# patrickltobing/cyclevae-vc

Measured on AMD Instinct MI355X. Metric: mcep_frames_per_sec_hu1024_ld32_cyc2, higher is better.
Workload: dtype f32 (every matrix product on exact fp32 operands: each operand carried as three fp16 limbs x = l0 + l1/2^11 + l2/2^22, six v_mfma_f32_32x32x16_f16 per product, f32 accumulate; dropped terms < 2^-33 of a product; gates, carried state, projection and outputs f32)

## Files before the change

cyclevae-vc_amd/csrc/cvae_kernels.h:

```cpp
#pragma once
#include <cvae_intrin.h>
#include <stdint.h>

struct CvaeSeg {
    const float* ptr;
    int width;
    int row_stride;
};

__device__ __forceinline__ void cvae_philox(uint32_t c0, uint32_t c1, uint32_t c2, uint32_t c3, uint32_t k0,
                                            uint32_t k1, uint32_t out[4]) {
    for (int i = 0; i < 10; ++i) {
        const uint64_t p0 = (uint64_t)0xD2511F53u * c0, p1 = (uint64_t)0xCD9E8D57u * c2;
        const uint32_t n0 = (uint32_t)(p1 >> 32) ^ c1 ^ k0, n1 = (uint32_t)p1;
        const uint32_t n2 = (uint32_t)(p0 >> 32) ^ c3 ^ k1, n3 = (uint32_t)p0;
        c0 = n0; c1 = n1; c2 = n2; c3 = n3;
        k0 += 0x9E3779B9u; k1 += 0xBB67AE85u;
    }
    out[0] = c0; out[1] = c1; out[2] = c2; out[3] = c3;
}

__device__ __forceinline__ void cvae_randn_pair(uint32_t w0, uint32_t w1, float& zc, float& zs) {
    const float u1 = ((float)(w0 >> 8) + 0.5f) * (1.0f / 16777216.0f);
    const float u2 = ((float)(w1 >> 8) + 0.5f) * (1.0f / 16777216.0f);
// ... 165 lines not shown
#define CVAE_MAX_CELLS 32
struct ProParams {
    ProCell cell[CVAE_MAX_CELLS];
    int ncell, L;
    uint64_t frame0;
    const float* sin_w;
    const float* sin_b;
    const float* wo;
    const float* bo;
    int B, T, C, Cp, pad, Co, H, Bp, nslack, nzero;
    long mtot;
    float* xnp;
    float* hbuf;
    float* hx;
    float* xt;
    int nxt_slack;
    float* hs;
    float* xs;
    long xs_plane;
    float* dy;
    unsigned* zero_words;
    int* zero_status;
    int zero_status_n;
    unsigned* ll_counter;
    int nA, nH, nD;
    int nG;
    float* gx0;
    const float* wyT;
    int* range_word;
    int* range_epoch;
    int range_val;
    float range_at;
    const int* image_unfit;
};
#ifndef CVAE_STATUS_RANGE_WORD
#define CVAE_STATUS_RANGE_WORD 3
#endif
#define CVAE_WS_RANGE_WORD 20
#define CVAE_WS_RANGE_EPOCH 21
#define CVAE_LIMB_MAX 65504.0f
__device__ __forceinline__ bool cvae_out_of_range(float v, float bound) { return !(fabsf(v) < bound); }
__device__ __forceinline__ void cvae_flag_unfit(int* unfit, float w) {
    if (cvae_out_of_range(w, CVAE_LIMB_MAX)) *unfit = 1;
}
static_assert(sizeof(ProParams) <= 4096, "ProParams is a kernel argument: 4 KiB at most");

__device__ __forceinline__ float cvae_input_value(const ProParams& p, const ProCell& c, int b, int t, int q, const float* emean = nullptr) {
    const long fr = (long)b * p.T + t;
    if (q < c.seg0.width) return c.seg0.ptr[fr * c.seg0.row_stride + q];
    if (!c.lat) return c.seg1.ptr[fr * c.seg1.row_stride + (q - c.seg0.width)];
    const int l = q - c.seg0.width;
    float e;
    if (c.n_draws > 1 && emean) {
        e = emean[l];
    } else if (c.n_draws > 1) {
        e = 0.0f;
        const long es = c.eps_stride ? c.eps_stride : (long)p.B * p.T * p.L;
        for (int k = 0; k < c.n_draws; ++k)
            e += c.eps ? c.eps[(long)k * es + fr * p.L + l]
                       : cvae_randn(c.seed, c.draw + (uint64_t)k, (uint64_t)(fr + c.draw_frame0) + p.frame0, (uint32_t)l);
        e *= 1.0f / (float)c.n_draws;
    } else {
        e = c.eps ? c.eps[fr * p.L + l] : cvae_randn(c.seed, c.draw, (uint64_t)(fr + c.draw_frame0) + p.frame0, (uint32_t)l);
    }
    return c.lat[fr * 2 * p.L + l] + expf(c.lat[fr * 2 * p.L + p.L + l] * 0.5f) * e;
}

__device__ __forceinline__ void cvae_mean_draws(const ProParams& p, const ProCell& c, int b, int t, float* part, float* emean) {
    const int tid = threadIdx.x, L = p.L, nq = L >> 2, nsl = 256 / nq, qd = tid % nq, sl = tid / nq;
    const long fr = (long)b * p.T + t;
    const long es = c.eps_stride ? c.eps_stride : (long)p.B * p.T * p.L;
    if (sl < nsl) {
        float e[4] = {0.f, 0.f, 0.f, 0.f};
        for (int k = sl; k < c.n_draws; k += nsl) {
            float z[4];
            if (c.eps) {
                const float* ep = c.eps + (long)k * es + fr * p.L + 4 * qd;
                z[0] = ep[0]; z[1] = ep[1]; z[2] = ep[2]; z[3] = ep[3];
            } else {
                cvae_randn4(c.seed, c.draw + (uint64_t)k, (uint64_t)(fr + c.draw_frame0) + p.frame0, (uint32_t)qd, z);
            }
#pragma unroll
            for (int j = 0; j < 4; ++j) e[j] += z[j];
        }
#pragma unroll
        for (int j = 0; j < 4; ++j) part[sl * L + 4 * qd + j] = e[j];
    }
    __syncthreads();
    if (tid < L) {
        float m = 0.0f;
        for (int q = 0; q < nsl; ++q) m += part[q * L + tid];
        emean[tid] = m * (1.0f / (float)c.n_draws);
    }
    __syncthreads();
}

__global__ void k_prologue(ProParams p) {
    const int tid = threadIdx.x, blk = blockIdx.x;
    const int Tp = p.T + 2 * p.pad;
    if (blk < p.nA && p.xt) {
        float* raw = (float*)CVAE_SMEM;
        unsigned char* img = (unsigned char*)(raw + 32 * (p.C + 1));
        const int tile = blk / Tp, tp = blk % Tp, t = tp - p.pad, np = p.Cp >> 3;
        float* tmean = (float*)(img + np * 1280);
        const bool quads = p.L > 0 && (p.L & 3) == 0;
        if (quads) {
            const int nq = p.L >> 2;
            for (int item = tid; item < 32 * nq; item += 256) {
                const int r = item / nq, qd = item - r * nq, bb = tile * 32 + r;
                if (bb >= p.ncell * p.B) continue;
                const ProCell& c = p.cell[bb / p.B];
                if (!c.lat || c.n_draws <= 1 || !CVAE_FRAME_VALID(p, c, t)) continue;
                const long fr = (long)(bb % p.B) * p.T + t, es = c.eps_stride ? c.eps_stride : (long)p.B * p.T * p.L;
                float e[4] = {0.f, 0.f, 0.f, 0.f};
                for (int k = 0; k < c.n_draws; ++k) {
                    float z[4];
                    if (c.eps) {
                        const float* ep = c.eps + (long)k * es + fr * p.L + 4 * qd;
                        z[0] = ep[0]; z[1] = ep[1]; z[2] = ep[2]; z[3] = ep[3];
                    } else {
                        cvae_randn4(c.seed, c.draw + (uint64_t)k, (uint64_t)(fr + c.draw_frame0) + p.frame0, (uint32_t)qd, z);
                    }
#pragma unroll
                    for (int j = 0; j < 4; ++j) e[j] += z[j];
                }
#pragma unroll
                for (int j = 0; j < 4; ++j) tmean[r * p.L + 4 * qd + j] = e[j] * (1.0f / (float)c.n_draws);
            }
            __syncthreads();
        }
        for (int idx = tid; idx < 32 * p.C; idx += 256) {
            const int r = idx / p.C, q = idx - r * p.C, bb = tile * 32 + r;
            float v = 0.0f;
            if (bb < p.ncell * p.B) {
                const ProCell& c = p.cell[bb / p.B];
                if (CVAE_FRAME_VALID(p, c, t)) v = cvae_input_value(p, c, bb % p.B, t, q, quads ? tmean + r * p.L : nullptr);
            }
            raw[r * (p.C + 1) + q] = v;
        }
        __syncthreads();
        const ProCell* const cells = p.cell;
        bool bad = false;
        for (int q = tid & 63; q < p.Cp; q += 64) {
            float v[8];
            bool ok[8];
#pragma unroll
            for (int i = 0; i < 8; ++i) {
                const int r = (tid >> 6) + 4 * i, bb = tile * 32 + r;
                ok[i] = false;
                if (bb < p.ncell * p.B) {
                    const ProCell& c = cells[bb / p.B];
                    ok[i] = CVAE_FRAME_VALID(p, c, t) && q < p.C;
                }
                v[i] = !ok[i] ? 0.0f : (p.sin_w ? p.sin_b[q] : raw[r * (p.C + 1) + q]);
            }
            if (p.sin_w && q < p.C)
                for (int k = 0; k < p.C; ++k) {
                    const float w = p.sin_w[(long)q * p.C + k];
#pragma unroll
                    for (int i = 0; i < 8; ++i) v[i] += w * raw[((tid >> 6) + 4 * i) * (p.C + 1) + k];
                }
            unsigned char* pc = img + (q >> 3) * 1280;
#pragma unroll
            for (int i = 0; i < 8; ++i) {
                const int r = (tid >> 6) + 4 * i;
                unsigned short l0, l1;
                unsigned char l2;
                cvae_split3_f16b8(ok[i] ? v[i] : 0.0f, l0, l1, l2);
                bad = bad || (ok[i] && cvae_out_of_range(v[i], p.range_at));
                ((unsigned short*)pc)[r * 8 + (q & 7)] = l0;
                ((unsigned short*)(pc + 512))[r * 8 + (q & 7)] = l1;
                pc[1024 + r * 8 + (q & 7)] = l2;
            }
        }
        const bool fits = cvae_block_all(!bad);
        if (!fits && p.range_word && tid == 0) *p.range_word = p.range_val;
        f32x4* dst = (f32x4*)((unsigned char*)p.xt + ((long)tile * Tp + tp) * np * 1280);
        for (int e = tid; e < np * 80; e += 256) dst[e] = ((const f32x4*)img)[e];
        return;
    }
    if (p.nG > 0 && blk >= p.nA + p.nH + p.nD && blk < p.nA + p.nH + p.nD + p.nG) {
        const long q4 = ((long)(blk - p.nA - p.nH - p.nD) * blockDim.x + tid) * 4, H3 = 3L * p.H;
        if (q4 < (long)p.ncell * p.B * H3) {
            const int bb = (int)(q4 / H3), col = (int)(q4 - (long)bb * H3);
            const float* yi = p.cell[bb / p.B].y_in + (long)(bb % p.B) * p.Co;
            float a0 = 0.f, a1 = 0.f, a2 = 0.f, a3 = 0.f;
            int c = 0;
            for (; c + 8 <= p.Co; c += 8) {
                float d[8], w[8][4];
#pragma unroll
                for (int q = 0; q < 8; ++q) {
                    d[q] = yi[c + q] - p.bo[c + q];
                    const float* wp = p.wyT + (long)(c + q) * H3 + col;
                    w[q][0] = wp[0]; w[q][1] = wp[1]; w[q][2] = wp[2]; w[q][3] = wp[3];
                }
#pragma unroll
                for (int q = 0; q < 8; ++q) { a0 += w[q][0] * d[q]; a1 += w[q][1] * d[q]; a2 += w[q][2] * d[q]; a3 += w[q][3] * d[q]; }
            }
            for (; c < p.Co; ++c) {
                const float d = yi[c] - p.bo[c];
                const float* w = p.wyT + (long)c * H3 + col;
                a0 += w[0] * d; a1 += w[1] * d; a2 += w[2] * d; a3 += w[3] * d;
            }
            float* o = p.gx0 + (long)bb * H3 + col;
            o[0] = a0; o[1] = a1; o[2] = a2; o[3] = a3;
        }
        return;
    }
    const float* emean = nullptr;
    if (blk < p.nA && blockDim.x == 256) {
        const int tp = blk % Tp, bb = blk / Tp, t = tp - p.pad;
        if (bb < p.ncell * p.B) {
            const ProCell& c = p.cell[bb / p.B];
            if (c.lat && c.n_draws > 1 && p.L <= 256 && (p.L & 3) == 0 && CVAE_FRAME_VALID(p, c, t)) {
                float* part = (float*)CVAE_SMEM + p.C;
// ... 1040 lines not shown
```

cyclevae-vc_amd/csrc/cvae_lib.hip:

```cpp
#include <cvae_intrin.h>

#include <stdarg.h>
#include <stdio.h>
#include <stdlib.h>
#include <string.h>

#include <atomic>
#include <map>
#include <mutex>
#include <new>
#include <utility>
#include <vector>

#include "cvae_kernels.h"
#include "cvae_train_kernels.h"
#include "cvae_deep.h"
#include "cyclevae_hip.h"

namespace {

thread_local char g_err[512] = "";

enum OptId {
    OPT_V6_LIMBS_H64, OPT_NO_LL, OPT_MAX_RT, OPT_LL_BACKOFF, OPT_EXP, OPT_GEMM_FORCE, OPT_GEMM_LOG, OPT_TRAIN_OLD_GEMM,
    OPT_GEMM_TRACE, OPT_TRAIN_PER_STEP, OPT_TRAIN_PROF, OPT_TRAIN_BACKOFF, OPT_TRAIN_FP32_MFMA, OPT_TRAIN_BWD_PER_STEP, OPT_TRAIN_KERNEL, OPT_X3_TILE, OPT_BWD_OVERFLOW_AT, OPT_GEMM_MAX_SPLIT, OPT_BWD_KS, OPT_COOP_LAUNCH, OPT_V6_LIMBS_H2048, OPT_V6_W2S_H64, OPT_STEP_COL_TILES, OPT_TRAIN_PROFILE, OPT_TRAIN_XMAP, OPT_MASKS_ON_SIDE, OPT_V6_BACKOFF, OPT_TRAIN_BWD_BACKOFF, OPT_LL_ROW_PAD, OPT_GEMM_MIN_DEPTH, OPT_TRAIN_BWD_GEOM, OPT_BWD_W3_L1_H64, OPT_TRAIN_FWD_GEOM, OPT_TRAIN_FWD_BACKOFF, OPT_EXACT_RANGE_AT, OPT_DTW_BATCH_COST, OPT_COUNT
};
struct OptEntry { const char* name; long dflt; };
const OptEntry g_opt[OPT_COUNT] = {
    {"v6_limbs_h64", 3},
    {"no_ll", 0},
    {"max_rt", 0},
    {"ll_backoff", -1},
    {"exp", 0},
    {"gemm_force", 0},
    {"gemm_log", 0},
    {"train_old_gemm", 0},
    {"gemm_trace", 0},
    {"train_per_step", 0},
    {"train_prof", 0},
    {"train_backoff", 32},
    {"train_fp32_mfma", 0},
    {"train_bwd_per_step", 0},
    {"train_kernel", 0},
    {"x3_tile", 0},
    {"bwd_overflow_at", 60000},
    {"gemm_max_split", 16},
    {"bwd_ks", 8},
    {"coop_launch", 0},
    {"v6_limbs_h2048", 3},
    {"v6_w2s_h64", 0},
    {"step_col_tiles", 0},
    {"train_profile", 0},
    {"train_xmap", 0},
    {"masks_on_side", 1},
    {"v6_backoff", -1},
    {"train_bwd_backoff", -1},
    {"ll_row_pad", 0},
    {"gemm_min_depth", 128},
    {"train_bwd_geom", -1},
    {"bwd_w3_l1_h64", 0},
    {"train_fwd_geom", -1},
    {"train_fwd_backoff", -1},
    {"exact_range_at", 65504},
    {"dtw_batch_cost", 1},
};

struct ProfEvents {
    std::vector<hipEvent_t> start, stop;
    std::vector<int> rows, cin;
    size_t used = 0;
};
enum { TPROF_FWD = 0, TPROF_BWD = 1, TPROF_GEMM = 2, TPROF_WGRAD = 3, TPROF_CLASSES = 4 };
struct TrainProfEvents {
    std::vector<hipEvent_t> start, stop;
    std::vector<int> cls;
    std::vector<double> flop;
    size_t used = 0;
};
struct SideDone { const void* scratch; hipEvent_t ev; };

}

struct cvae_ctx {
    int32_t* status_sink = nullptr;
    long draw_row0 = 0, draw_rows = 0, draw_frames = 0, draw_parts = 1;
    long opt[OPT_COUNT];
    ProfEvents prof;
    TrainProfEvents tprof;
    hipStream_t side = nullptr;
    SideDone side_done[8] = {};
    hipEvent_t side_ready = nullptr, side_join = nullptr, side_last = nullptr;
    int side_cap = 0;
    hipEvent_t mask_fork = nullptr, mask_join = nullptr;
    unsigned side_evict = 0;
    int32_t* gemm_ran = nullptr;
    std::map<const void*, std::pair<int, unsigned long>> train_var;
    unsigned long train_var_tick = 0;
// ... 416 lines not shown
        const cvae_pass_input* in = cells[c].in;
        const int w_in = in->seg0.width + (in->lat ? in->lat_dim : in->seg1.width);
        if (w_in != m.C) return fail(-1, "cell %d: pass input width %d != in_dim %d", c, w_in, m.C);
        if (in->frames < 0 || in->frames > T) return fail(-1, "cell %d: frames %d outside [0, T=%d]", c, in->frames, T);
        if (in->ctx_before < 0 || in->ctx_after < 0 || in->draw_frame0 < 0 || in->eps_draw_stride < 0)
            return fail(-1, "cell %d: negative window context / draw origin", c);
        if ((in->ctx_before || in->ctx_after || in->draw_frame0) && B != 1)
            return fail(-1, "cell %d: windows of a longer utterance (ctx_before / ctx_after / draw_frame0) are single-row cells, B=%d", c, B);
    }
    return 0;
}

struct ProTargets {
    int shape;
    float* xnp;
    float* dy;
    float* slot0;
    unsigned* zero_words;
    int nzero;
    int* zero_status;
    int zero_status_n;
    int* ws_status;
    bool limbs, new_call;
    float* hx;
    float* xt;
    int nxt_slack;
    float* hs;
    float* xs;
    long xs_plane;
    float* gx0;
    unsigned* ll_counter;
};
struct RangeSlot { int* word; int val; float at; };

void run_prologue(const Dims& m, const cvae_net_desc* d, const float* P, const Prep& pl, const PassRows& r, const ProTargets& o,
                  hipStream_t st, RangeSlot* range = nullptr) {
    const Cell* cells = r.cells;
    const int ncell = r.ncell, B = r.B, T = r.T, Bp = r.Bp, shape = o.shape;
    const int Brows = ncell * B, Tp = T + 2 * m.pad;
    ProParams pp;
    memset(&pp, 0, sizeof(pp));
    for (int c = 0; c < ncell; ++c) {
        const cvae_pass_input* in = cells[c].in;
        pp.cell[c].seg0 = CvaeSeg{in->seg0.ptr, in->seg0.width, in->seg0.row_stride};
        pp.cell[c].seg1 = CvaeSeg{in->seg1.ptr, in->seg1.width, in->seg1.row_stride};
        pp.cell[c].lat = in->lat;
        pp.cell[c].eps = in->eps;
        pp.cell[c].seed = in->seed;
        pp.cell[c].draw = in->draw_id;
        pp.cell[c].y_in = cells[c].y_in;
        pp.cell[c].h_in = cells[c].h_in;
        pp.cell[c].frames = in->frames;
        pp.cell[c].n_draws = in->n_draws;
        pp.cell[c].ctx_before = in->ctx_before; pp.cell[c].ctx_after = in->ctx_after;
        pp.cell[c].draw_frame0 = (long)in->draw_frame0; pp.cell[c].eps_stride = (long)in->eps_draw_stride;
        if (in->lat) pp.L = in->lat_dim;
    }
    pp.ncell = ncell;
    pp.frame0 = (uint64_t)cx().draw_row0 * (uint64_t)T;
    pp.sin_w = d->has_scale_in ? P + pl.sin_w : nullptr;
    pp.sin_b = d->has_scale_in ? P + pl.sin_b : nullptr;
    pp.wo = P + pl.wo; pp.bo = P + pl.bo;
    pp.B = B; pp.T = T; pp.C = m.C; pp.Cp = m.Cp; pp.pad = m.pad; pp.Co = m.Co; pp.H = m.H; pp.Bp = Bp;
    pp.nslack = 64 * m.KFW + 64;
    pp.mtot = r.mtot;
    pp.xnp = o.xnp; pp.hbuf = o.slot0; pp.dy = o.dy;
    pp.hx = o.hx; pp.xt = o.xt; pp.nxt_slack = o.nxt_slack;
    pp.hs = o.hs; pp.xs = o.xs; pp.xs_plane = o.xs_plane;
    pp.zero_words = o.zero_words; pp.nzero = o.nzero;
    pp.zero_status = o.zero_status; pp.zero_status_n = o.zero_status_n;
    pp.ll_counter = o.ll_counter;
    pp.nA = (shape == PRO_TILES ? Bp / 32 : Brows) * Tp;
    pp.nH = (int)nblk((long)Bp * m.H, 1024);
    pp.nD = (int)nblk((long)Brows * m.Co, 64);
    pp.nG = o.gx0 ? (int)nblk((long)Brows * m.H3 / 4, shape == PRO_ROWS ? 64 : 256) : 0;
    pp.gx0 = o.gx0; pp.wyT = P + pl.wyT;
    range_params(pp, o.ws_status, o.limbs, o.new_call, P, pl);
    if (range) *range = RangeSlot{pp.range_word, pp.range_val, pp.range_at};
    const dim3 gp(pp.nA + pp.nH + pp.nD + pp.nG + 1);
    if (shape == PRO_TILES)
        hipLaunchKernelGGL((k_prologue), gp, dim3(256),
                           (size_t)32 * (m.C + 1) * sizeof(float) + (size_t)(m.Cp / 8) * 1280 + (size_t)32 * pp.L * sizeof(float), st, pp);
    else if (shape == PRO_DRAWS)
        hipLaunchKernelGGL((k_prologue), gp, dim3(256), (size_t)(m.C + 1024 + 256) * sizeof(float), st, pp);
    else
        hipLaunchKernelGGL((k_prologue), gp, dim3(64), m.C * sizeof(float), st, pp);
}

void run_front_end_gemm(const Dims& m, const float* P, const Prep& pl, const float* xnp, float* gx, int rows, int Tp, hipStream_t st) {
    const int M = rows * Tp, N = m.H3;
    hipLaunchKernelGGL((k_gemm_nt<4, 4, 2, 2, false>), dim3(nblk(N, 128), nblk(M, 128)), dim3(256), 0, st, xnp, (long)m.Cp, 0L,
                       P + pl.afold, (long)m.Kfe, P + pl.cfold, gx, (long)m.H3, M, N, m.Kfe);
}

void run_projection(const Dims& m, const cvae_net_desc* d, const float* P, const Prep& pl, const PassRows& r, int proj, const float* hbuf,
                    float* y, int clamp_lat_dim, hipStream_t st) {
    const Cell* cells = r.cells;
    const int ncell = r.ncell, B = r.B, T = r.T, Bp = r.Bp;
    const long mtot = r.mtot;
    if (proj == PROJ_FUSED) {
        OutParams op;
        op.hbuf = hbuf; op.mtot = mtot; op.wo2 = P + pl.wo2; op.bo2 = P + pl.bo2; op.H = m.H; op.Bp = Bp; op.T = T;
        op.B = B; op.ncell = ncell; op.Co = m.Co; op.clamp_from = d->has_scale_out ? -1 : clamp_dim(clamp_lat_dim);
        op.clamp_min = clamp_floor(clamp_lat_dim);
        for (int c = 0; c < CVAE_MAX_CELLS; ++c) op.out[c] = c < ncell ? cells[c].trj_out : nullptr;
        const int ntn = m.Cop / 16;
        const unsigned nb = (unsigned)((long)T * Bp / 16);
        const size_t lds = (size_t)4 * 16 * (m.Cop + 4) * sizeof(float);
        void (*const kout)(OutParams) = ntn == 1 ? k_outproj<1> : ntn == 4 ? k_outproj<4> : k_outproj<8>;
        hipLaunchKernelGGL(kout, dim3(nb), dim3(256), lds, st, op);
        return;
    }
    const int M = T * Bp, N = m.Co;
    hipLaunchKernelGGL((k_gemm_nt<2, 4, 4, 1, true>), dim3(nblk(N, 64), nblk(M, 128)), dim3(256), 0, st, hbuf + (long)Bp * 16, 0L, mtot,
                       P + pl.wo, (long)m.H, P + pl.bo, y, (long)m.Cop, M, N, m.H);
    for (int c = 0; c < ncell; ++c) {
        EpiParams ep;
        ep.y = y; ep.ldy = m.Cop;
        ep.sout_w = d->has_scale_out ? P + pl.sout_w : nullptr;
        ep.sout_b = d->has_scale_out ? P + pl.sout_b : nullptr;
        ep.clamp_from = d->has_scale_out ? -1 : clamp_dim(clamp_lat_dim);
        ep.clamp_min = clamp_floor(clamp_lat_dim);
        ep.B = B; ep.Bp = Bp; ep.T = T; ep.Co = m.Co; ep.b0 = c * B;
        ep.trj_out = cells[c].trj_out; ep.y_last = cells[c].y_last;
        ep.t_last = last_slot(cells[c].in, T) - 1;
        hipLaunchKernelGGL((k_epilogue), dim3(B * T), dim3(64), m.Co * sizeof(float), st, ep);
    }
}

void run_last_states(const Dims& m, const PassRows& r, const float* hbuf, hipStream_t st) {
    for (int c = 0; c < r.ncell; ++c)
        if (r.cells[c].h_last)
            hipLaunchKernelGGL((k_hlast), dim3(nblk((long)r.B * m.H, 256)), dim3(256), 0, st, hbuf, r.mtot, r.cells[c].h_last, r.B, r.Bp,
                               m.H, last_slot(r.cells[c].in, r.T), c * r.B);
}

int run_pass(const Dims& m, const cvae_net_desc* d, const float* P, const Cell* cells, int ncell, int B, int T,
             int clamp_lat_dim, float* ws, int* status, int flags, hipStream_t st, bool clear_status = false) {
    const Prep pl = prep_layout(m, d->has_scale_in != 0, d->has_scale_out != 0);
    const int Brows = ncell * B;
    const Work wl = work_layout(m, Brows, T);
    int* const ws_status = status;
    if (cx().status_sink) status = cx().status_sink;
    const PassRows rows = {cells, ncell, B, T, wl.Bp, wl.mtot};
    if (int rc = check_cells(m, rows)) return rc;
    unsigned* bar = (unsigned*)(ws + wl.status) + 8;
    float* xnp = ws + wl.xnp;
    float* gx = ws + wl.gx;
    float* hbuf = ws + wl.hbuf;
    float* dy = ws + wl.dy;
    unsigned* hflags = (unsigned*)(ws + wl.flags);
    long long* const step_prof = (flags & CVAE_FLAG_STEP_TIMING) ? (long long*)(ws + wl.prof) : nullptr;
    const int cus = cu_count();
    PassFacts facts = {};
    for (int c = 0; c < ncell; ++c) {
        facts.h_in = facts.h_in || cells[c].h_in != nullptr;
        facts.y_last = facts.y_last || cells[c].y_last != nullptr;
        facts.h_last = facts.h_last || cells[c].h_last != nullptr;
        facts.many_draws = facts.many_draws || (cells[c].in->lat && cells[c].in->n_draws > 1);
    }
    const EvalPlan pn = plan_eval_pass(m, Brows, T, flags, cus, image_known_unfit(P), facts);

    {
        ProTargets o = {};
        o.shape = pn.prologue; o.xnp = xnp; o.dy = dy;
        o.slot0 = hbuf;
        o.zero_words = hflags; o.nzero = wl.Bp / 16 * m.nch;
        o.zero_status = clear_status ? status : nullptr;
        o.zero_status_n = cx().status_sink ? 4 : 8;
        o.ws_status = ws_status; o.limbs = pn.limbs; o.new_call = clear_status;
        const bool triples = pn.form == CVAE_EVAL_V6 || pn.form == CVAE_EVAL_V6H;
        o.hx = triples ? ws + wl.hs : nullptr;
        o.xt = pn.form == CVAE_EVAL_V6 ? ws + wl.xt : nullptr;
        o.nxt_slack = (int)wl.xt_slack;
        o.hs = pn.pairs ? ws + wl.hs : nullptr;
        o.xs = pn.pairs ? ws + wl.xs : nullptr;
        o.xs_plane = wl.xs_plane;
        o.gx0 = pn.gx0_ready ? ws + wl.gx0 : nullptr;
        o.ll_counter = pn.form == CVAE_EVAL_LL ? (unsigned*)(ws + wl.status) + 16 : nullptr;
        run_prologue(m, d, P, pl, rows, o, st);
    }

    const size_t lds2 = (4 * 16 * 84 + 16 * 16) * sizeof(float);
    const bool prof = (flags & CVAE_FLAG_PROFILE) && prof_begin(st, ncell * B, m.C);
    const auto refused = [](hipError_t e) {
        if (e == hipSuccess) return false;
        (void)hipGetLastError();
        return true;
    };
    int form = pn.form;
    if (form == CVAE_EVAL_LL || form == CVAE_EVAL_V6H || form <= CVAE_EVAL_V2) run_front_end_gemm(m, P, pl, xnp, gx, Brows, wl.Tp, st);
    switch (form) {
    case CVAE_EVAL_LL: {
        StepLLParams q;
        q.hbuf = hbuf; q.mtot = wl.mtot; q.xbuf = ws + wl.hs; q.wrec2 = P + pl.wrec2; q.gx = gx; q.gx_bstride = (long)wl.Tp * m.H3;
        q.bhn = P + pl.bhn; q.B = Brows; q.Bp = wl.Bp; q.H = m.H; q.T = T; q.status = status;
        q.prof = step_prof;
        q.wyT = P + pl.wyT; q.dy = dy; q.Co = m.Co;
        q.dbg = (int*)(ws + wl.status);
        q.backoff = pn.backoff;
        q.nonce_src = (const unsigned*)(ws + wl.status) + 16;
        const dim3 gl(m.H / 4);
        const size_t ldsl = (size_t)(2 * 64 * 49 + 4 * 48) * sizeof(float);
        const hipError_t e = cvae_launch_coop(Brows == 1 ? k_gru_steps_ll<1> : Brows == 2 ? k_gru_steps_ll<2> : k_gru_steps_ll<3>, gl,
                                              dim3(256), ldsl, st, q);
        if (refused(e)) return fail(-3, "small-batch recurrent kernel failed to launch: %s", hipGetErrorString(e));
        break;
    }
    case CVAE_EVAL_V6:
    case CVAE_EVAL_V6H: {
        const bool fused = form == CVAE_EVAL_V6;
        Step6Params q;
        q.hbuf = hbuf; q.mtot = wl.mtot; q.hx = ws + wl.hs; q.wrec3 = P + pl.wrec_t; q.afold3 = fused ? P + pl.afold_t : nullptr; q.w2s = P + pl.wrec_l2b;
        q.cfold = P + pl.cfold; q.bhn = P + pl.bhn; q.xt = fused ? ws + wl.xt : nullptr; q.Tp = wl.Tp; q.Cp = m.Cp;
        q.gx = fused ? nullptr : gx; q.gx_bstride = (long)wl.Tp * m.H3;
        q.B = Brows; q.Bp = wl.Bp; q.H = m.H; q.T = T; q.flags = hflags; q.status = status;
        q.prof = step_prof;
        q.wyT = P + pl.wyT; q.dy = dy; q.Co = m.Co;
        q.gx0 = pn.gx0_ready ? ws + wl.gx0 : nullptr;
        q.want_f32 = pn.want_f32 ? 1 : 0;
        q.rts = pn.rts;
        q.exp = (int)opt(OPT_EXP);
        q.backoff = pn.backoff;
        const size_t lds6 = (size_t)(4 * 32 * 40 + 32 * 8 + 384 + (fused ? 4 * m.KFW * v6_limbs(m) * 256 : 0)) * sizeof(float);
        const hipError_t e = cvae_launch_coop(pn.k6, dim3(m.H / 8 * pn.rts), dim3(256), lds6, st, q);
        if (refused(e)) return fail(-3, "exact-operand recurrent kernel failed to launch: %s", hipGetErrorString(e));
        break;
    }
    case CVAE_EVAL_V5:
    case CVAE_EVAL_V4: {
        Step3Params q;
        q.hbuf = hbuf; q.mtot = wl.mtot; q.wrec2 = P + pl.wrec2; q.cfold = P + pl.cfold;
        q.xnp = xnp; q.Tp = wl.Tp; q.Cp = m.Cp; q.bhn = P + pl.bhn; q.B = Brows; q.Bp = wl.Bp; q.H = m.H; q.T = T;
        q.flags = hflags; q.status = status;
        q.prof = step_prof;
        q.wyT = P + pl.wyT; q.dy = dy; q.Co = m.Co;
        q.rts = pn.rts;
        q.hs = ws + wl.hs; q.wrec_h = P + pl.wrec_h; q.xs = ws + wl.xs; q.xs_plane = wl.xs_plane;
        q.exp = (int)opt(OPT_EXP);
        const dim3 g(m.nch * pn.rts);
        if (form == CVAE_EVAL_V5) {
            q.afold2 = P + pl.afold_h;
            const size_t lds5 = lds2 + (size_t)4 * ((m.KFW + 1) / 2) * 6 * 256 * sizeof(float);
            if (!refused(cvae_launch_coop(pn.k5, g, dim3(256), lds5, st, q))) break;
        }
        q.afold2 = P + pl.afold3;
        const size_t lds4 = lds2 + (size_t)4 * m.KFW * 3 * 256 * sizeof(float);
        if (!refused(cvae_launch_coop(pn.k4, g, dim3(256), lds4, st, q))) break;
        run_front_end_gemm(m, P, pl, xnp, gx, Brows, wl.Tp, st);
        form = CVAE_EVAL_V2;
    }
        [[fallthrough]];
// ... 324 lines not shown
int cvae_sample(cvae_ctx* ctx, const float* lat, int rows, int lat_dim, const float* eps, uint64_t seed, uint64_t draw_id, float* z,
                float* eps_out, void* stream) {
    CVAE_ENTER(ctx);
    if (!lat || !z || rows < 0 || lat_dim < 1) return fail(-1, "bad argument");
    if (rows == 0) return 0;
    hipLaunchKernelGGL((k_sample), dim3(nblk((long)rows * lat_dim, 256)), dim3(256), 0, (hipStream_t)stream, lat, rows,
                       lat_dim, eps, seed, draw_id, z, eps_out, (uint64_t)cx().draw_row0 * (uint64_t)cx().draw_frames);
    CVAE_HIP_OK(hipGetLastError());
    return 0;
}

int cvae_sample_laplace(cvae_ctx* ctx, const float* lat, int rows, int lat_dim, const float* eps, uint64_t seed, uint64_t draw_id,
                        float* z, float* eps_out, void* stream) {
    CVAE_ENTER(ctx);
    if (!lat || !z || rows < 0 || lat_dim < 1) return fail(-1, "bad argument");
    if (rows == 0) return 0;
    hipLaunchKernelGGL((k_sample_laplace), dim3(nblk((long)rows * lat_dim, 256)), dim3(256), 0, (hipStream_t)stream, lat, rows,
                       lat_dim, eps, seed, draw_id, z, eps_out, (uint64_t)cx().draw_row0 * (uint64_t)cx().draw_frames);
    CVAE_HIP_OK(hipGetLastError());
    return 0;
}

int cvae_sample_laplace_backward(cvae_ctx* ctx, const float* dz, const float* lat, const float* z, int rows, int lat_dim, float* dlat,
                                 void* stream) {
    CVAE_ENTER(ctx);
    if (!dz || !lat || !z || !dlat || rows < 0 || lat_dim < 1) return fail(-1, "bad argument");
    if (rows == 0) return 0;
    hipLaunchKernelGGL((k_sample_laplace_bwd), dim3(nblk((long)rows * lat_dim, 256)), dim3(256), 0, (hipStream_t)stream, dz, lat, z,
                       rows, lat_dim, dlat);
    CVAE_HIP_OK(hipGetLastError());
    return 0;
}

static long cycle_layout(const Dims& me, const Dims& md, int B, int T, long* pass_off, long* traj_off) {
    const long pe = work_layout(me, B, T).total, pd = work_layout(md, 2 * B, T).total;
    long o = 64;
    *pass_off = o;
    o += pe > pd ? pe : pd;
    *traj_off = o;
    o += up((long)B * T * me.Co, 64) * 2 + up((long)B * T * md.Co, 64) * 3;
    return o;
}

size_t cvae_cycle_workspace_bytes(cvae_ctx* ctx, const cvae_net_desc* enc, const cvae_net_desc* dec, int B, int T, int n_cyc) {
    CVAE_ENTER_SZ(ctx);
    Dims me, md;
    if (make_dims(enc, &me) || make_dims(dec, &md) || B < 1 || T < 1 || n_cyc < 1) return 0;
    long po, to;
    return (size_t)cycle_layout(me, md, B, T, &po, &to) * sizeof(float);
}

static int cycle_forward_impl(const cvae_net_desc* enc, const void* enc_prepared, const cvae_net_desc* dec,
                       const void* dec_prepared, const float* x, const float* cvx, int stdim, const float* code_src,
                       const float* code_trg, int ncode, const float* y_in_enc, const float* y_in_dec, int B, int T,
                       int n_cyc, int lat_dim, const float* eps, uint64_t seed, float* out_lat, float* out_rec,
                       float* out_cv, float* out_latcv, float* out_reccyc, void* workspace, size_t workspace_bytes,
                       int flags, void* stream, const cvae_cycle_state* sin, const cvae_cycle_state* sout) {
    Dims me, md;
    if (int rc = make_dims(enc, &me)) return rc;
    if (int rc = make_dims(dec, &md)) return rc;
    if (B < 1 || T < 1 || n_cyc < 1) return fail(-1, "empty work: B=%d T=%d n_cyc=%d", B, T, n_cyc);
    if (!enc_prepared || !dec_prepared || !x || !cvx || !code_src || !code_trg || !y_in_enc || !y_in_dec || !workspace)
        return fail(-1, "null argument");
    if (me.Co != 2 * lat_dim) return fail(-1, "encoder out_dim %d != 2*lat_dim %d", me.Co, 2 * lat_dim);
    if (md.C != ncode + lat_dim) return fail(-1, "decoder in_dim %d != ncode+lat_dim %d", md.C, ncode + lat_dim);
    if (me.C != stdim + md.Co) return fail(-1, "encoder in_dim %d != stdim+decoder out_dim %d", me.C, stdim + md.Co);
    if (workspace_bytes < cvae_cycle_workspace_bytes(tl_ctx, enc, dec, B, T, n_cyc)) return fail(-2, "workspace too small");
    hipStream_t st = (hipStream_t)stream;
    float* ws = (float*)workspace;
    long po, to;
    cycle_layout(me, md, B, T, &po, &to);
    float* pws = ws + po;
    const long ne = (long)B * T * me.Co, nd = (long)B * T * md.Co;
    float* t_lat = ws + to;
    float* t_latcv = t_lat + up(ne, 64);
    float* t_rec = t_latcv + up(ne, 64);
    float* t_cv = t_rec + up(nd, 64);
    float* t_reccyc = t_cv + up(nd, 64);
    const float* prev_reccyc = nullptr;
    int* status = (int*)workspace;
    const long neps = (long)B * T * lat_dim;
    if (sin && (!sin->y_enc || !sin->y_dec || !sin->h_enc || !sin->h_dec)) return fail(-1, "incomplete input cycle state");
    if (sout && (!sout->y_enc || !sout->y_dec || !sout->h_enc || !sout->h_dec)) return fail(-1, "incomplete output cycle state");
    auto ye = [&](const cvae_cycle_state* s, int i, int slot) { return s ? s->y_enc + ((long)i * 2 + slot) * B * me.Co : nullptr; };
    auto he = [&](const cvae_cycle_state* s, int i, int slot) { return s ? s->h_enc + ((long)i * 2 + slot) * B * me.H : nullptr; };
    auto yd = [&](const cvae_cycle_state* s, int i, int slot) { return s ? s->y_dec + ((long)i * 3 + slot) * B * md.Co : nullptr; };
    auto hd = [&](const cvae_cycle_state* s, int i, int slot) { return s ? s->h_dec + ((long)i * 3 + slot) * B * md.H : nullptr; };

    for (int i = 0; i < n_cyc; ++i) {
        float* lat = out_lat ? out_lat + i * ne : t_lat;
        float* latcv = out_latcv ? out_latcv + i * ne : t_latcv;
        float* rec = out_rec ? out_rec + i * nd : t_rec;
        float* cv = out_cv ? out_cv + i * nd : t_cv;
        float* reccyc = out_reccyc ? out_reccyc + i * nd : t_reccyc;
        cvae_pass_input in, in2;
        memset(&in, 0, sizeof(in));
        int rc;
        if (i == 0) {
            in.seg0 = cvae_seg{x, me.C, me.C};
        } else {
            in.seg0 = cvae_seg{x, stdim, me.C};
            in.seg1 = cvae_seg{prev_reccyc, md.Co, md.Co};
        }
        {
            const Cell c{&in, sin ? ye(sin, i, 0) : y_in_enc, he(sin, i, 0), lat, ye(sout, i, 0), he(sout, i, 0)};
            if ((rc = run_pass(me, enc, (const float*)enc_prepared, &c, 1, B, T, lat_dim, pws, status, flags, st, i == 0))) return rc;
        }
        memset(&in, 0, sizeof(in));
        in.seg0 = cvae_seg{code_src, ncode, ncode};
        in.lat = lat; in.lat_dim = lat_dim;
        in.eps = eps ? eps + (i * 3 + 0) * neps : nullptr;
        in.seed = seed; in.draw_id = (uint64_t)(i * 3 + 0);
        in2 = in;
        in2.seg0 = cvae_seg{code_trg, ncode, ncode};
        in2.eps = eps ? eps + (i * 3 + 1) * neps : nullptr;
        in2.draw_id = (uint64_t)(i * 3 + 1);
        {
            const Cell c2[2] = {{&in, sin ? yd(sin, i, 0) : y_in_dec, hd(sin, i, 0), rec, yd(sout, i, 0), hd(sout, i, 0)},
                                {&in2, sin ? yd(sin, i, 1) : y_in_dec, hd(sin, i, 1), cv, yd(sout, i, 1), hd(sout, i, 1)}};
            if ((rc = run_pass(md, dec, (const float*)dec_prepared, c2, 2, B, T, -1, pws, status, flags, st))) return rc;
        }
        memset(&in, 0, sizeof(in));
        in.seg0 = cvae_seg{cvx, stdim, stdim};
        in.seg1 = cvae_seg{cv, md.Co, md.Co};
        {
            const Cell c{&in, sin ? ye(sin, i, 1) : y_in_enc, he(sin, i, 1), latcv, ye(sout, i, 1), he(sout, i, 1)};
            if ((rc = run_pass(me, enc, (const float*)enc_prepared, &c, 1, B, T, lat_dim, pws, status, flags, st))) return rc;
        }
        memset(&in, 0, sizeof(in));
        in.seg0 = cvae_seg{code_src, ncode, ncode};
        in.lat = latcv; in.lat_dim = lat_dim;
        in.eps = eps ? eps + (i * 3 + 2) * neps : nullptr;
        in.seed = seed; in.draw_id = (uint64_t)(i * 3 + 2);
        {
            const Cell c{&in, sin ? yd(sin, i, 2) : y_in_dec, hd(sin, i, 2), reccyc, yd(sout, i, 2), hd(sout, i, 2)};
            if ((rc = run_pass(md, dec, (const float*)dec_prepared, &c, 1, B, T, -1, pws, status, flags, st))) return rc;
        }
        prev_reccyc = reccyc;
    }
    return 0;
}

int cvae_cycle_forward(cvae_ctx* ctx, const cvae_net_desc* enc, const void* enc_prepared, const cvae_net_desc* dec,
                       const void* dec_prepared, const float* x, const float* cvx, int stdim, const float* code_src,
                       const float* code_trg, int ncode, const float* y_in_enc, const float* y_in_dec, int B, int T,
                       int n_cyc, int lat_dim, const float* eps, uint64_t seed, float* out_lat, float* out_rec,
                       float* out_cv, float* out_latcv, float* out_reccyc, void* workspace, size_t workspace_bytes,
                       int flags, void* stream) {
    CVAE_ENTER(ctx);
    return cycle_forward_impl(enc, enc_prepared, dec, dec_prepared, x, cvx, stdim, code_src, code_trg, ncode, y_in_enc, y_in_dec,
                              B, T, n_cyc, lat_dim, eps, seed, out_lat, out_rec, out_cv, out_latcv, out_reccyc, workspace,
                              workspace_bytes, flags, stream, nullptr, nullptr);
}

int cvae_cycle_forward_carry(cvae_ctx* ctx, const cvae_net_desc* enc, const void* enc_prepared, const cvae_net_desc* dec,
                             const void* dec_prepared, const float* x, const float* cvx, int stdim, const float* code_src,
                             const float* code_trg, int ncode, const float* y_in_enc, const float* y_in_dec, int B, int T,
                             int n_cyc, int lat_dim, const float* eps, uint64_t seed, float* out_lat, float* out_rec,
                             float* out_cv, float* out_latcv, float* out_reccyc, void* workspace, size_t workspace_bytes,
                             int flags, void* stream, const cvae_cycle_state* state_in, const cvae_cycle_state* state_out) {
    CVAE_ENTER(ctx);
    return cycle_forward_impl(enc, enc_prepared, dec, dec_prepared, x, cvx, stdim, code_src, code_trg, ncode, y_in_enc, y_in_dec,
                              B, T, n_cyc, lat_dim, eps, seed, out_lat, out_rec, out_cv, out_latcv, out_reccyc, workspace,
                              workspace_bytes, flags, stream, state_in, state_out);
}

int cvae_step_timing(cvae_ctx* ctx, const cvae_net_desc* d, int B, int T, const void* workspace, double out[8], void* stream) {
    CVAE_ENTER(ctx);
    Dims m;
// ... 108 lines not shown
```

Before: 1.332 million.

## Rework prologue input loads, vectorize noise draws, and share initial gate projection across cycle passes

The prologue now generates single-draw latent noise four at a time with randn4 into shared memory. It batches the input gathers eight per thread so loads are issued before the exp/combine work. The gx0 (initial y_in projection) kernel computes four rows per thread to reuse weight loads. In the cycle forward path, gx0 buffers are kept per encoder and decoder across passes and skipped after the first pass, since y_in is constant when no state input is given. This adds workspace and a correctness dependence on y_in and weights staying unchanged within a call.

Result: no change. 1.337 million, median of 6 (+0.4%).

```diff
diff --git a/cyclevae-vc_amd/csrc/cvae_kernels.h b/cyclevae-vc_amd/csrc/cvae_kernels.h
--- a/cyclevae-vc_amd/csrc/cvae_kernels.h
+++ b/cyclevae-vc_amd/csrc/cvae_kernels.h
@@ -221,7 +221,12 @@
     int range_val;
     float range_at;
     const int* image_unfit;
+    int form;
 };
+#define PRO_FORM_LOADS 1
+#define PRO_FORM_QUADS 2
+#define PRO_FORM_GX0 4
+#define PRO_GX0_ROWS 4
 #ifndef CVAE_STATUS_RANGE_WORD
 #define CVAE_STATUS_RANGE_WORD 3
 #endif
@@ -234,7 +239,16 @@
 }
 static_assert(sizeof(ProParams) <= 4096, "ProParams is a kernel argument: 4 KiB at most");
 
-__device__ __forceinline__ float cvae_input_value(const ProParams& p, const ProCell& c, int b, int t, int q, const float* emean = nullptr) {
+__device__ __forceinline__ float cvae_fmac(float w, float x, float acc) {
+#if defined(__HIP_DEVICE_COMPILE__)
+    return __builtin_fmaf(w, x, acc);
+#else
+    return acc + w * x;
+#endif
+}
+
+__device__ __forceinline__ float cvae_input_value(const ProParams& p, const ProCell& c, int b, int t, int q, const float* emean = nullptr,
+                                                  const float* zq = nullptr) {
     const long fr = (long)b * p.T + t;
     if (q < c.seg0.width) return c.seg0.ptr[fr * c.seg0.row_stride + q];
     if (!c.lat) return c.seg1.ptr[fr * c.seg1.row_stride + (q - c.seg0.width)];
@@ -250,7 +264,8 @@
                        : cvae_randn(c.seed, c.draw + (uint64_t)k, (uint64_t)(fr + c.draw_frame0) + p.frame0, (uint32_t)l);
         e *= 1.0f / (float)c.n_draws;
     } else {
-        e = c.eps ? c.eps[fr * p.L + l] : cvae_randn(c.seed, c.draw, (uint64_t)(fr + c.draw_frame0) + p.frame0, (uint32_t)l);
+        e = c.eps ? c.eps[fr * p.L + l]
+                  : (zq ? zq[l] : cvae_randn(c.seed, c.draw, (uint64_t)(fr + c.draw_frame0) + p.frame0, (uint32_t)l));
     }
     return c.lat[fr * 2 * p.L + l] + expf(c.lat[fr * 2 * p.L + p.L + l] * 0.5f) * e;
 }
@@ -284,7 +299,7 @@
     __syncthreads();
 }
 
-__global__ void k_prologue(ProParams p) {
+__global__ __launch_bounds__(256) void k_prologue(ProParams p) {
     const int tid = threadIdx.x, blk = blockIdx.x;
     const int Tp = p.T + 2 * p.pad;
     if (blk < p.nA && p.xt) {
@@ -292,15 +307,24 @@
         unsigned char* img = (unsigned char*)(raw + 32 * (p.C + 1));
         const int tile = blk / Tp, tp = blk % Tp, t = tp - p.pad, np = p.Cp >> 3;
         float* tmean = (float*)(img + np * 1280);
-        const bool quads = p.L > 0 && (p.L & 3) == 0;
+        const bool quads = p.L > 0 && (p.L & 3) == 0, zquads = quads && (p.form & PRO_FORM_QUADS);
         if (quads) {
             const int nq = p.L >> 2;
             for (int item = tid; item < 32 * nq; item += 256) {
                 const int r = item / nq, qd = item - r * nq, bb = tile * 32 + r;
                 if (bb >= p.ncell * p.B) continue;
                 const ProCell& c = p.cell[bb / p.B];
-                if (!c.lat || c.n_draws <= 1 || !CVAE_FRAME_VALID(p, c, t)) continue;
+                if (!c.lat || !CVAE_FRAME_VALID(p, c, t)) continue;
                 const long fr = (long)(bb % p.B) * p.T + t, es = c.eps_stride ? c.eps_stride : (long)p.B * p.T * p.L;
+                if (c.n_draws <= 1) {
+                    if (zquads && !c.eps) {
+                        float z[4];
+                        cvae_randn4(c.seed, c.draw, (uint64_t)(fr + c.draw_frame0) + p.frame0, (uint32_t)qd, z);
+#pragma unroll
+                        for (int j = 0; j < 4; ++j) tmean[r * p.L + 4 * qd + j] = z[j];
+                    }
+                    continue;
+                }
                 float e[4] = {0.f, 0.f, 0.f, 0.f};
                 for (int k = 0; k < c.n_draws; ++k) {
                     float z[4];
@@ -318,12 +342,39 @@
             }
             __syncthreads();
         }
-        for (int idx = tid; idx < 32 * p.C; idx += 256) {
+        for (int base = 0; (p.form & PRO_FORM_LOADS) && base < 32 * p.C; base += 8 * 256) {
+            float va[8], vb[8], ve[8];
+            int kind[8];
+#pragma unroll
+            for (int it = 0; it < 8; ++it) {
+                const int idx = base + it * 256 + tid, r = idx / p.C, q = idx - r * p.C, bb = tile * 32 + r;
+                va[it] = 0.0f; vb[it] = 0.0f; ve[it] = 0.0f; kind[it] = 0;
+                if (idx >= 32 * p.C || bb >= p.ncell * p.B) continue;
+                const ProCell& c = p.cell[bb / p.B];
+                if (!CVAE_FRAME_VALID(p, c, t)) continue;
+                const long fr = (long)(bb % p.B) * p.T + t;
+                const int l = q - c.seg0.width;
+                if (q < c.seg0.width) va[it] = c.seg0.ptr[fr * c.seg0.row_stride + q];
+                else if (!c.lat) va[it] = c.seg1.ptr[fr * c.seg1.row_stride + l];
+                else if (c.n_draws <= 1 && (c.eps || zquads)) {
+                    kind[it] = 1;
+                    va[it] = c.lat[fr * 2 * p.L + l];
+                    vb[it] = c.lat[fr * 2 * p.L + p.L + l];
+                    ve[it] = c.eps ? c.eps[fr * p.L + l] : tmean[r * p.L + l];
+                } else va[it] = cvae_input_value(p, c, bb % p.B, t, q, quads ? tmean + r * p.L : nullptr, zquads ? tmean + r * p.L : nullptr);
+            }
+#pragma unroll
+            for (int it = 0; it < 8; ++it) {
+                const int idx = base + it * 256 + tid, r = idx / p.C, q = idx - r * p.C;
+                if (idx < 32 * p.C) raw[r * (p.C + 1) + q] = kind[it] ? va[it] + expf(vb[it] * 0.5f) * ve[it] : va[it];
+            }
+        }
+        for (int idx = tid; !(p.form & PRO_FORM_LOADS) && idx < 32 * p.C; idx += 256) {
             const int r = idx / p.C, q = idx - r * p.C, bb = tile * 32 + r;
             float v = 0.0f;
             if (bb < p.ncell * p.B) {
                 const ProCell& c = p.cell[bb / p.B];
-                if (CVAE_FRAME_VALID(p, c, t)) v = cvae_input_value(p, c, bb % p.B, t, q, quads ? tmean + r * p.L : nullptr);
+                if (CVAE_FRAME_VALID(p, c, t)) v = cvae_input_value(p, c, bb % p.B, t, q, quads ? tmean + r * p.L : nullptr, zquads ? tmean + r * p.L : nullptr);
             }
             raw[r * (p.C + 1) + q] = v;
         }
@@ -343,12 +394,13 @@
                 }
                 v[i] = !ok[i] ? 0.0f : (p.sin_w ? p.sin_b[q] : raw[r * (p.C + 1) + q]);
             }
-            if (p.sin_w && q < p.C)
+            if (p.sin_w && q < p.C) {
                 for (int k = 0; k < p.C; ++k) {
                     const float w = p.sin_w[(long)q * p.C + k];
 #pragma unroll
                     for (int i = 0; i < 8; ++i) v[i] += w * raw[((tid >> 6) + 4 * i) * (p.C + 1) + k];
                 }
+            }
             unsigned char* pc = img + (q >> 3) * 1280;
 #pragma unroll
             for (int i = 0; i < 8; ++i) {
@@ -370,6 +422,53 @@
     }
     if (p.nG > 0 && blk >= p.nA + p.nH + p.nD && blk < p.nA + p.nH + p.nD + p.nG) {
         const long q4 = ((long)(blk - p.nA - p.nH - p.nD) * blockDim.x + tid) * 4, H3 = 3L * p.H;
+        if (p.form & PRO_FORM_GX0) {
+            const int rows = p.ncell * p.B, ngrp = (rows + PRO_GX0_ROWS - 1) / PRO_GX0_ROWS;
+            if (q4 >= (long)ngrp * H3) return;
+            const int grp = (int)(q4 / H3), col = (int)(q4 - (long)grp * H3);
+            const float* yi[PRO_GX0_ROWS];
+            float a[PRO_GX0_ROWS][4];
+#pragma unroll
+            for (int r = 0; r < PRO_GX0_ROWS; ++r) {
+                const int bb = grp * PRO_GX0_ROWS + r < rows ? grp * PRO_GX0_ROWS + r : rows - 1;
+                yi[r] = p.cell[bb / p.B].y_in + (long)(bb % p.B) * p.Co;
+                a[r][0] = a[r][1] = a[r][2] = a[r][3] = 0.f;
+            }
+            int c = 0;
+            for (; c + 8 <= p.Co; c += 8) {
+                float d[PRO_GX0_ROWS][8], w[8][4];
+#pragma unroll
+                for (int q = 0; q < 8; ++q) {
+                    const float* wp = p.wyT + (long)(c + q) * H3 + col;
+                    w[q][0] = wp[0]; w[q][1] = wp[1]; w[q][2] = wp[2]; w[q][3] = wp[3];
+#pragma unroll
+                    for (int r = 0; r < PRO_GX0_ROWS; ++r) d[r][q] = yi[r][c + q] - p.bo[c + q];
+                }
+#pragma unroll
+                for (int q = 0; q < 8; ++q)
+#pragma unroll
+                    for (int r = 0; r < PRO_GX0_ROWS; ++r) {
+#pragma unroll
+                        for (int e = 0; e < 4; ++e) a[r][e] = cvae_fmac(w[q][e], d[r][q], a[r][e]);
+                    }
+            }
+            for (; c < p.Co; ++c) {
+                const float* w = p.wyT + (long)c * H3 + col;
+#pragma unroll
+                for (int r = 0; r < PRO_GX0_ROWS; ++r) {
+                    const float d = yi[r][c] - p.bo[c];
+#pragma unroll
+                    for (int e = 0; e < 4; ++e) a[r][e] = cvae_fmac(w[e], d, a[r][e]);
+                }
+            }
+#pragma unroll
+            for (int r = 0; r < PRO_GX0_ROWS; ++r)
+                if (grp * PRO_GX0_ROWS + r < rows) {
+                    float* o = p.gx0 + (long)(grp * PRO_GX0_ROWS + r) * H3 + col;
+                    o[0] = a[r][0]; o[1] = a[r][1]; o[2] = a[r][2]; o[3] = a[r][3];
+                }
+            return;
+        }
         if (q4 < (long)p.ncell * p.B * H3) {
             const int bb = (int)(q4 / H3), col = (int)(q4 - (long)bb * H3);
             const float* yi = p.cell[bb / p.B].y_in + (long)(bb % p.B) * p.Co;
diff --git a/cyclevae-vc_amd/csrc/cvae_lib.hip b/cyclevae-vc_amd/csrc/cvae_lib.hip
--- a/cyclevae-vc_amd/csrc/cvae_lib.hip
+++ b/cyclevae-vc_amd/csrc/cvae_lib.hip
@@ -23,7 +23,7 @@
 
 enum OptId {
     OPT_V6_LIMBS_H64, OPT_NO_LL, OPT_MAX_RT, OPT_LL_BACKOFF, OPT_EXP, OPT_GEMM_FORCE, OPT_GEMM_LOG, OPT_TRAIN_OLD_GEMM,
-    OPT_GEMM_TRACE, OPT_TRAIN_PER_STEP, OPT_TRAIN_PROF, OPT_TRAIN_BACKOFF, OPT_TRAIN_FP32_MFMA, OPT_TRAIN_BWD_PER_STEP, OPT_TRAIN_KERNEL, OPT_X3_TILE, OPT_BWD_OVERFLOW_AT, OPT_GEMM_MAX_SPLIT, OPT_BWD_KS, OPT_COOP_LAUNCH, OPT_V6_LIMBS_H2048, OPT_V6_W2S_H64, OPT_STEP_COL_TILES, OPT_TRAIN_PROFILE, OPT_TRAIN_XMAP, OPT_MASKS_ON_SIDE, OPT_V6_BACKOFF, OPT_TRAIN_BWD_BACKOFF, OPT_LL_ROW_PAD, OPT_GEMM_MIN_DEPTH, OPT_TRAIN_BWD_GEOM, OPT_BWD_W3_L1_H64, OPT_TRAIN_FWD_GEOM, OPT_TRAIN_FWD_BACKOFF, OPT_EXACT_RANGE_AT, OPT_DTW_BATCH_COST, OPT_COUNT
+    OPT_GEMM_TRACE, OPT_TRAIN_PER_STEP, OPT_TRAIN_PROF, OPT_TRAIN_BACKOFF, OPT_TRAIN_FP32_MFMA, OPT_TRAIN_BWD_PER_STEP, OPT_TRAIN_KERNEL, OPT_X3_TILE, OPT_BWD_OVERFLOW_AT, OPT_GEMM_MAX_SPLIT, OPT_BWD_KS, OPT_COOP_LAUNCH, OPT_V6_LIMBS_H2048, OPT_V6_W2S_H64, OPT_STEP_COL_TILES, OPT_TRAIN_PROFILE, OPT_TRAIN_XMAP, OPT_MASKS_ON_SIDE, OPT_V6_BACKOFF, OPT_TRAIN_BWD_BACKOFF, OPT_LL_ROW_PAD, OPT_GEMM_MIN_DEPTH, OPT_TRAIN_BWD_GEOM, OPT_BWD_W3_L1_H64, OPT_TRAIN_FWD_GEOM, OPT_TRAIN_FWD_BACKOFF, OPT_EXACT_RANGE_AT, OPT_DTW_BATCH_COST, OPT_PROLOGUE_FORM, OPT_COUNT
 };
 struct OptEntry { const char* name; long dflt; };
 const OptEntry g_opt[OPT_COUNT] = {
@@ -63,6 +63,7 @@
     {"train_fwd_backoff", -1},
     {"exact_range_at", 65504},
     {"dtw_batch_cost", 1},
+    {"prologue_form", 7},
 };
 
 struct ProfEvents {
@@ -545,6 +546,7 @@
     unsigned* ll_counter;
 };
 struct RangeSlot { int* word; int val; float at; };
+struct ChainGx0 { float* buf; int rows; };
 
 void run_prologue(const Dims& m, const cvae_net_desc* d, const float* P, const Prep& pl, const PassRows& r, const ProTargets& o,
                   hipStream_t st, RangeSlot* range = nullptr) {
@@ -586,7 +588,9 @@
     pp.nA = (shape == PRO_TILES ? Bp / 32 : Brows) * Tp;
     pp.nH = (int)nblk((long)Bp * m.H, 1024);
     pp.nD = (int)nblk((long)Brows * m.Co, 64);
-    pp.nG = o.gx0 ? (int)nblk((long)Brows * m.H3 / 4, shape == PRO_ROWS ? 64 : 256) : 0;
+    pp.form = (int)opt(OPT_PROLOGUE_FORM);
+    const long grows = (pp.form & PRO_FORM_GX0) ? (Brows + PRO_GX0_ROWS - 1) / PRO_GX0_ROWS : Brows;
+    pp.nG = o.gx0 ? (int)nblk(grows * m.H3 / 4, shape == PRO_ROWS ? 64 : 256) : 0;
     pp.gx0 = o.gx0; pp.wyT = P + pl.wyT;
     range_params(pp, o.ws_status, o.limbs, o.new_call, P, pl);
     if (range) *range = RangeSlot{pp.range_word, pp.range_val, pp.range_at};
@@ -649,7 +653,7 @@
 }
 
 int run_pass(const Dims& m, const cvae_net_desc* d, const float* P, const Cell* cells, int ncell, int B, int T,
-             int clamp_lat_dim, float* ws, int* status, int flags, hipStream_t st, bool clear_status = false) {
+             int clamp_lat_dim, float* ws, int* status, int flags, hipStream_t st, bool clear_status = false, ChainGx0* chain = nullptr) {
     const Prep pl = prep_layout(m, d->has_scale_in != 0, d->has_scale_out != 0);
     const int Brows = ncell * B;
     const Work wl = work_layout(m, Brows, T);
@@ -673,6 +677,10 @@
         facts.many_draws = facts.many_draws || (cells[c].in->lat && cells[c].in->n_draws > 1);
     }
     const EvalPlan pn = plan_eval_pass(m, Brows, T, flags, cus, image_known_unfit(P), facts);
+    const bool chain_gx0 = chain && pn.gx0_ready;
+    const bool gx0_formed = chain_gx0 && chain->rows >= Brows;
+    float* const gx0 = !pn.gx0_ready ? nullptr : (chain_gx0 ? chain->buf : ws + wl.gx0);
+    if (chain_gx0 && !gx0_formed) chain->rows = Brows;
 
     {
         ProTargets o = {};
@@ -689,7 +697,7 @@
         o.hs = pn.pairs ? ws + wl.hs : nullptr;
         o.xs = pn.pairs ? ws + wl.xs : nullptr;
         o.xs_plane = wl.xs_plane;
-        o.gx0 = pn.gx0_ready ? ws + wl.gx0 : nullptr;
+        o.gx0 = gx0_formed ? nullptr : gx0;
         o.ll_counter = pn.form == CVAE_EVAL_LL ? (unsigned*)(ws + wl.status) + 16 : nullptr;
         run_prologue(m, d, P, pl, rows, o, st);
     }
@@ -730,7 +738,7 @@
         q.B = Brows; q.Bp = wl.Bp; q.H = m.H; q.T = T; q.flags = hflags; q.status = status;
         q.prof = step_prof;
         q.wyT = P + pl.wyT; q.dy = dy; q.Co = m.Co;
-        q.gx0 = pn.gx0_ready ? ws + wl.gx0 : nullptr;
+        q.gx0 = gx0;
         q.want_f32 = pn.want_f32 ? 1 : 0;
         q.rts = pn.rts;
         q.exp = (int)opt(OPT_EXP);
@@ -1121,13 +1129,17 @@
     return 0;
 }
 
-static long cycle_layout(const Dims& me, const Dims& md, int B, int T, long* pass_off, long* traj_off) {
+static long cycle_layout(const Dims& me, const Dims& md, int B, int T, long* pass_off, long* traj_off, long* gx0_off = nullptr) {
     const long pe = work_layout(me, B, T).total, pd = work_layout(md, 2 * B, T).total;
     long o = 64;
     *pass_off = o;
     o += pe > pd ? pe : pd;
     *traj_off = o;
     o += up((long)B * T * me.Co, 64) * 2 + up((long)B * T * md.Co, 64) * 3;
+    if (gx0_off) gx0_off[0] = o;
+    o += up((long)B * me.H3, 64);
+    if (gx0_off) gx0_off[1] = o;
+    o += up(2L * B * md.H3, 64);
     return o;
 }
 
@@ -1157,9 +1169,13 @@
     if (workspace_bytes < cvae_cycle_workspace_bytes(tl_ctx, enc, dec, B, T, n_cyc)) return fail(-2, "workspace too small");
     hipStream_t st = (hipStream_t)stream;
     float* ws = (float*)workspace;
-    long po, to;
-    cycle_layout(me, md, B, T, &po, &to);
+    long po, to, go[2];
+    cycle_layout(me, md, B, T, &po, &to, go);
     float* pws = ws + po;
+    const bool share_gx0 = !sin && (opt(OPT_PROLOGUE_FORM) & PRO_FORM_GX0);
+    ChainGx0 ge = {ws + go[0], 0}, gd = {ws + go[1], 0};
+    ChainGx0* const cge = share_gx0 ? &ge : nullptr;
+    ChainGx0* const cgd = share_gx0 ? &gd : nullptr;
     const long ne = (long)B * T * me.Co, nd = (long)B * T * md.Co;
     float* t_lat = ws + to;
     float* t_latcv = t_lat + up(ne, 64);
@@ -1193,7 +1209,7 @@
         }
         {
             const Cell c{&in, sin ? ye(sin, i, 0) : y_in_enc, he(sin, i, 0), lat, ye(sout, i, 0), he(sout, i, 0)};
-            if ((rc = run_pass(me, enc, (const float*)enc_prepared, &c, 1, B, T, lat_dim, pws, status, flags, st, i == 0))) return rc;
+            if ((rc = run_pass(me, enc, (const float*)enc_prepared, &c, 1, B, T, lat_dim, pws, status, flags, st, i == 0, cge))) return rc;
         }
         memset(&in, 0, sizeof(in));
         in.seg0 = cvae_seg{code_src, ncode, ncode};
@@ -1207,14 +1223,14 @@
         {
             const Cell c2[2] = {{&in, sin ? yd(sin, i, 0) : y_in_dec, hd(sin, i, 0), rec, yd(sout, i, 0), hd(sout, i, 0)},
                                 {&in2, sin ? yd(sin, i, 1) : y_in_dec, hd(sin, i, 1), cv, yd(sout, i, 1), hd(sout, i, 1)}};
-            if ((rc = run_pass(md, dec, (const float*)dec_prepared, c2, 2, B, T, -1, pws, status, flags, st))) return rc;
+            if ((rc = run_pass(md, dec, (const float*)dec_prepared, c2, 2, B, T, -1, pws, status, flags, st, false, cgd))) return rc;
         }
         memset(&in, 0, sizeof(in));
         in.seg0 = cvae_seg{cvx, stdim, stdim};
         in.seg1 = cvae_seg{cv, md.Co, md.Co};
         {
             const Cell c{&in, sin ? ye(sin, i, 1) : y_in_enc, he(sin, i, 1), latcv, ye(sout, i, 1), he(sout, i, 1)};
-            if ((rc = run_pass(me, enc, (const float*)enc_prepared, &c, 1, B, T, lat_dim, pws, status, flags, st))) return rc;
+            if ((rc = run_pass(me, enc, (const float*)enc_prepared, &c, 1, B, T, lat_dim, pws, status, flags, st, false, cge))) return rc;
         }
         memset(&in, 0, sizeof(in));
         in.seg0 = cvae_seg{code_src, ncode, ncode};
@@ -1223,7 +1239,7 @@
         in.seed = seed; in.draw_id = (uint64_t)(i * 3 + 2);
         {
             const Cell c{&in, sin ? yd(sin, i, 2) : y_in_dec, hd(sin, i, 2), reccyc, yd(sout, i, 2), hd(sout, i, 2)};
-            if ((rc = run_pass(md, dec, (const float*)dec_prepared, &c, 1, B, T, -1, pws, status, flags, st))) return rc;
+            if ((rc = run_pass(md, dec, (const float*)dec_prepared, &c, 1, B, T, -1, pws, status, flags, st, false, cgd))) return rc;
         }
         prev_reccyc = reccyc;
     }
```
